# egorchistov/color-transfer

Hardware: AMD Instinct MI355X
Metric: stereopairs/s at 1920×1080 (linear + dcmcs3di fwd), 1/2/4/8 GPU (higher is better)
Workload: dtype f32 (float32 I/O; float32 difference forms in both sweeps, float64 only in the per-frame statistics records)

## Files before the change

### color-transfer_amd/csrc/reinhard_persist.hip

```cpp
#include <atomic>
#include <mutex>

#include "ct_reinhard.h"
#include "ct_reinhard_persist.h"

namespace ct {
namespace rp {

#ifndef CT_RP_ILP
#define CT_RP_ILP 1
#endif
#define CT_RP_PIXEL_FENCE(q) do { if (((q) + 1) % CT_RP_ILP == 0) __builtin_amdgcn_sched_barrier(0); } while (0)

#ifndef CT_RP_F32_WAVES
#define CT_RP_F32_WAVES 16
#endif
constexpr int kMaxWaves = 16;
constexpr int kTileBytes = kTilePixels * 12;
constexpr int kShards = 8;
constexpr int kRecWords = 32;
constexpr int kDataWords = 24;
constexpr int kSlabWord = 24;
constexpr int kMaxPairs = 64;
constexpr int kErrBytes = 64;

constexpr uint64_t kValMask = (1ull << 52) - 1;
constexpr int kInvShift = 52, kCntShift = 58;
constexpr double kHiScale = 0x1p24, kLoScale = 0x1p40;
constexpr int64_t kHiBias = 1ll << 46;

struct Scratch {
    double red[2][kMaxWaves][12];
    double coef[2][8];
    double side[kMaxWaves][6];
    double tot[12];
    double stat[2][CT_LAB_STATS_STRIDE];
    double fin[12 * 8];
    unsigned long long rec[kShards * kDataWords];
    float piv[2 * kMaxPairs][4];
    float lut255[256];
    float lin255f[256];
    unsigned cnt[2];
    unsigned ticket[3];
    unsigned ready[2];
    int flag[2];
};
constexpr int kLdsFixed = lut::kLdsBytesAll + (int)sizeof(Scratch);
constexpr int kLdsMax = 160 * 1024;
constexpr int kMaxParked = (kLdsMax - kLdsFixed) / (2 * kTileBytes);
constexpr int kMaxSlots = 32 * kMaxWaves / 2;
static_assert(lut::kLdsBytesAll % 16 == 0 && kTileBytes % 16 == 0, "16-byte aligned LDS regions");

struct Args {
    const void *target, *reference, *gt;
    float *out;
    int64_t n_pixels;
    int batch, slots, pslots;
    unsigned long long *rec;
    double *slab;
    double *sq;
    unsigned *err;
    double *stats_t, *stats_r;
    unsigned long long *stamps;
};

__device__ __forceinline__ uint64_t realtime() { return __builtin_amdgcn_s_memrealtime(); }
constexpr uint64_t kSpinTicks = 200000000ull;
__device__ unsigned g_status;
__device__ __forceinline__ void give_up(unsigned *err) {
    __hip_atomic_store(err, 1u, __ATOMIC_RELAXED, __HIP_MEMORY_SCOPE_AGENT);
    (void)__hip_atomic_fetch_or(&g_status, 1u, __ATOMIC_RELAXED, __HIP_MEMORY_SCOPE_AGENT);
}

template <typename T> struct Tile;
template <> struct Tile<float> {
    struct Raw { float e[12]; };
    static __device__ __forceinline__ void load(const void *p, int lane, Raw &r) { load_tile(reinterpret_cast<const float *>(p), lane, r.e); }
    static __device__ __forceinline__ bool in_range(const Raw &r) { return __builtin_amdgcn_ballot_w64(max_bits12(r.e) > lut::kOneBits) == 0; }
};
template <> struct Tile<uint8_t> {
    struct Raw { uint32_t d[3]; };
    static __device__ __forceinline__ void load(const void *p, int lane, Raw &r) {
        const uint8_t *q = reinterpret_cast<const uint8_t *>(p) + lane * 12;
        if ((reinterpret_cast<uintptr_t>(p) & 3) == 0) {
            typedef uint32_t u3 __attribute__((ext_vector_type(3)));
            const u3 v = *reinterpret_cast<const u3 __attribute__((aligned(4))) *>(q);
            r.d[0] = v.x; r.d[1] = v.y; r.d[2] = v.z;
        } else {
#pragma unroll
            for (int i = 0; i < 3; ++i) r.d[i] = (uint32_t)q[4 * i] | ((uint32_t)q[4 * i + 1] << 8) | ((uint32_t)q[4 * i + 2] << 16) | ((uint32_t)q[4 * i + 3] << 24);
        }
    }
    static __device__ __forceinline__ bool in_range(const Raw &) { return true; }
};
__device__ __forceinline__ uint32_t byte_of(const uint32_t (&d)[3], int i) { return (d[i >> 2] >> (8 * (i & 3))) & 255u; }

template <typename T>
__device__ __forceinline__ void load_pixel(const T *p, double &r, double &g, double &b) {
    if constexpr (sizeof(T) == 4) { r = p[0]; g = p[1]; b = p[2]; }
    else { r = (float)p[0] / 255.0f; g = (float)p[1] / 255.0f; b = (float)p[2] / 255.0f; }
}
template <typename T> __device__ __forceinline__ int pixel_of(int lane, int q) { return sizeof(T) == 4 ? q * kWave + lane : lane * 4 + q; }

template <typename T>
__device__ __forceinline__ void exact_moments_tile(const T *tile, const float (&kf)[3], double *side, int lane) {
    const double kd[3] = {(double)kf[0], (double)kf[1], (double)kf[2]};
    double s[6] = {0.0, 0.0, 0.0, 0.0, 0.0, 0.0};
#pragma unroll 1
    for (int q = 0; q < 4; ++q) {
        double r, g, b, x, y, z;
        load_pixel<T>(tile + pixel_of<T>(lane, q) * 3, r, g, b);
        to_space<true>(r, g, b, x, y, z);
        accumulate<true>(s, kd, x, y, z);
    }
#pragma unroll 1
    for (int m = 0; m < 6; ++m) {
        const double v = wave_sum(s[m]);
        if (lane == 0) side[m] += v;
    }
}

template <typename T, bool PARK, bool STATS = true>
__device__ __forceinline__ bool fwd_tile(const unsigned char *tab, Scratch *sc, const void *tile, typename Tile<T>::Raw &cur, const float (&kf)[3],
                                         float (&sf)[6], uint32_t *slot, int w, int lane) {
    const bool raw = !Tile<T>::in_range(cur);
    if constexpr (sizeof(T) == 4) {
        if (raw) {
            if (STATS) exact_moments_tile<T>(reinterpret_cast<const T *>(tile), kf, &sc->side[w][0], lane);
            return true;
        }
    }
    bool near = false;
#pragma unroll
    for (int q = 0; q < 4; ++q) {
        float fy, dxy, dyz;
        if constexpr (!PARK) {
            if constexpr (sizeof(T) == 4) {
                lut::rgb_to_f_stats(tab, cur.e[3 * q], cur.e[3 * q + 1], cur.e[3 * q + 2], fy, dxy, dyz);
            } else {
                const float l[3] = {sc->lin255f[byte_of(cur.d, 3 * q)], sc->lin255f[byte_of(cur.d, 3 * q + 1)], sc->lin255f[byte_of(cur.d, 3 * q + 2)]};
                lut::lin_to_f_stats(tab, l, fy, dxy, dyz);
            }
        } else {
            if constexpr (sizeof(T) == 4) {
                near |= lut::rgb_to_f(tab, cur.e[3 * q], cur.e[3 * q + 1], cur.e[3 * q + 2], fy, dxy, dyz);
            } else {
                const float l[3] = {sc->lin255f[byte_of(cur.d, 3 * q)], sc->lin255f[byte_of(cur.d, 3 * q + 1)], sc->lin255f[byte_of(cur.d, 3 * q + 2)]};
                near |= lut::lin_to_f(tab, l, fy, dxy, dyz);
            }
        }
        if (STATS) {
            const float e0 = fy - kf[0], e1 = dxy - kf[1], e2 = dyz - kf[2];
            sf[0] += e0; sf[1] += e1; sf[2] += e2;
            sf[3] = fmaf(e0, e0, sf[3]); sf[4] = fmaf(e1, e1, sf[4]); sf[5] = fmaf(e2, e2, sf[5]);
        }
        if (PARK) {
            slot[(3 * q) * kWave + lane] = __float_as_uint(fy);
            slot[(3 * q + 1) * kWave + lane] = __float_as_uint(dxy);
            slot[(3 * q + 2) * kWave + lane] = __float_as_uint(dyz);
        }
        CT_RP_PIXEL_FENCE(q);
    }
    return PARK && __builtin_amdgcn_ballot_w64(near) != 0;
}

template <typename T> __device__ __forceinline__ void store_pixel(float *tile, int lane, int q, float r, float g, float b) {
#ifdef CT_NT_STORE
    if constexpr (sizeof(T) == 4) {
        __builtin_nontemporal_store(float3v{r, g, b}, reinterpret_cast<float3u *>(tile + pixel_of<T>(lane, q) * 3));
        return;
    }
#endif
    *reinterpret_cast<float3u *>(tile + pixel_of<T>(lane, q) * 3) = float3v{r, g, b};
}

template <typename T, bool HAS_GT>
__device__ __forceinline__ void apply_tile(const unsigned char *tab, const Scratch *sc, const uint32_t *slot, bool raw, bool coef_bad,
                                           const ReinhardCoef &c, const float (&cf)[6], const void *tgt_tile, const void *gt_tile,
                                           float *out_tile, const typename Tile<T>::Raw &gv, double &sq, int lane) {
    float e = 0.f;
    auto gt_of = [&](int i) -> float {
        if constexpr (sizeof(T) == 4) return gv.e[i]; else return sc->lut255[byte_of(gv.d, i)];
    };
    bool slow = raw || coef_bad;
    if (!slow) {
        bool near = false;
#pragma unroll
        for (int q = 0; q < 4; ++q) {
            const float fy = __uint_as_float(slot[(3 * q) * kWave + lane]), dxy = __uint_as_float(slot[(3 * q + 1) * kWave + lane]),
                        dyz = __uint_as_float(slot[(3 * q + 2) * kWave + lane]);
            const float gy = fmaf(cf[0], fy, cf[3]), dx = fmaf(cf[1], dxy, cf[4]), dz = fmaf(cf[2], dyz, cf[5]);
            float r, g, b;
            near |= lut::f_to_rgb_clip(tab, gy, dx, dz, r, g, b);
            store_pixel<T>(out_tile, lane, q, r, g, b);
            if (HAS_GT) {
                const float d0 = r - gt_of(3 * q), d1 = g - gt_of(3 * q + 1), d2 = b - gt_of(3 * q + 2);
                e = fmaf(d0, d0, e); e = fmaf(d1, d1, e); e = fmaf(d2, d2, e);
            }
            CT_RP_PIXEL_FENCE(q);
        }
        slow = __builtin_amdgcn_ballot_w64(near) != 0;
    }
    if (slow) {
        e = 0.f;
#pragma unroll 1
        for (int q = 0; q < 4; ++q) {
            const int px = pixel_of<T>(lane, q);
            double r, g, b;
            load_pixel<T>(reinterpret_cast<const T *>(tgt_tile) + px * 3, r, g, b);
            float o0, o1, o2;
            reinhard_pixel<float, false>(c, r, g, b, o0, o1, o2);
            *reinterpret_cast<float3u *>(out_tile + px * 3) = float3v{o0, o1, o2};
            if (HAS_GT) {
                double g0, g1, g2;
                load_pixel<T>(reinterpret_cast<const T *>(gt_tile) + px * 3, g0, g1, g2);
                const float d0 = o0 - (float)g0, d1 = o1 - (float)g1, d2 = o2 - (float)g2;
                e = fmaf(d0, d0, e); e = fmaf(d1, d1, e); e = fmaf(d2, d2, e);
            }
        }
    }
    if (HAS_GT) sq += (double)e;
}

__device__ __forceinline__ int collect(const unsigned long long *rec, int nwg, int lane, Scratch *sc, unsigned *err) {
    const uint64_t t0 = realtime();
    for (;;) {
        bool ok = true;
#pragma unroll
        for (int j = 0; j < 3; ++j) {
            const int idx = lane + kWave * j;
            const int shard = idx / kDataWords, q = idx - shard * kDataWords;
            const unsigned long long x = __hip_atomic_load(rec + shard * kRecWords + q, __ATOMIC_RELAXED, __HIP_MEMORY_SCOPE_AGENT);
            ok &= (x >> kCntShift) == (unsigned long long)((nwg - shard + kShards - 1) / kShards);
            sc->rec[idx] = x;
        }
        __threadfence_block();
        if (__builtin_amdgcn_ballot_w64(!ok) == 0) break;
        if (realtime() - t0 > kSpinTicks) { if (lane == 0) give_up(err); return 2; }
        __builtin_amdgcn_s_sleep(8);
    }
    unsigned long long val = 0, inv = 0;
    if (lane < kDataWords) {
#pragma unroll
        for (int s = 0; s < kShards; ++s) {
            const unsigned long long x = sc->rec[s * kDataWords + lane];
            val += x & kValMask;
            inv += (x >> kInvShift) & 63ull;
        }
    }
    double dv = (lane & 1) ? (double)val * 0x1p-64 : (double)((long long)val - (long long)nwg * kHiBias) * 0x1p-24;
    dv += __shfl_down(dv, 1, kWave);
    if (lane < kDataWords && !(lane & 1)) sc->tot[lane >> 1] = dv;
    __threadfence_block();
    return __builtin_amdgcn_ballot_w64(lane < kDataWords && inv != 0) ? 1 : 0;
}

__device__ __forceinline__ void finish_stats(Scratch *sc, int par, int pair, int batch, int64_t n_pixels, int lane, double *stats_t, double *stats_r) {
    const double n = (double)n_pixels;
    if (lane < 6) {
        const int img = lane / 3, ch = lane - 3 * img;
        const double s1 = sc->tot[img * 6 + ch], s2 = sc->tot[img * 6 + 3 + ch];
        const double k = (double)sc->piv[img ? batch + pair : pair][ch];
        const double m0 = s1 / n;
        const double var = fma(-s1, m0, s2) / n;
        const double scale = ch == 0 ? 116.0 : (ch == 1 ? 500.0 : 200.0);
        const double mean = ch == 0 ? fma(116.0, k + m0, -16.0) : scale * (k + m0);
        const double sd = scale * var_to_sd(var, kVarFloorF32);
        sc->stat[img][ch] = mean;
        sc->stat[img][3 + ch] = sd;
        if (ch == 0) { sc->stat[img][6] = n; sc->stat[img][7] = 0.0; }
    }
    __threadfence_block();
    if (lane < 3) {
        const double mt = sc->stat[0][lane], st = sc->stat[0][3 + lane], mr = sc->stat[1][lane], sr = sc->stat[1][3 + lane];
        const double s = sr / st;
        double off;
        if (lane == 0) off = (fma(-16.0 - mt, s, mr) + 16.0) * (1.0 / 116.0);
        else off = fma(-mt, s, mr) * (lane == 1 ? 1.0 / 500.0 : 1.0 / 200.0);
        sc->coef[par][lane] = s;
        sc->coef[par][3 + lane] = off;
    }
    if (stats_t != nullptr && lane < 2 * CT_LAB_STATS_STRIDE) {
        const int img = lane / CT_LAB_STATS_STRIDE, m = lane - img * CT_LAB_STATS_STRIDE;
        (img ? stats_r : stats_t)[(size_t)pair * CT_LAB_STATS_STRIDE + m] = sc->stat[img][m];
    }
}

__device__ __forceinline__ float uniform_f32(float v) { return __uint_as_float(__builtin_amdgcn_readfirstlane(__float_as_uint(v))); }

template <typename T>
__device__ __forceinline__ void tail_moments(const T *p, int tail, const float (&kf)[3], Scratch *sc, int w, int lane) {
    if (w * kWave >= tail) return;
    double s[6] = {0.0, 0.0, 0.0, 0.0, 0.0, 0.0};
    const int t = w * kWave + lane;
    if (t < tail) {
        const double kd[3] = {(double)kf[0], (double)kf[1], (double)kf[2]};
        double x, y, z, r0, r1, r2;
        if constexpr (sizeof(T) == 4) { r0 = p[t * 3]; r1 = p[t * 3 + 1]; r2 = p[t * 3 + 2]; }
        else { r0 = (float)p[t * 3] / 255.0f; r1 = (float)p[t * 3 + 1] / 255.0f; r2 = (float)p[t * 3 + 2] / 255.0f; }
        to_space<true>(r0, r1, r2, x, y, z);
        accumulate<true>(s, kd, x, y, z);
    }
#pragma unroll 1
    for (int m = 0; m < 6; ++m) {
        const double v = wave_sum(s[m]);
        if (lane == 0) sc->side[w][m] += v;
    }
}

template <typename T, bool HAS_GT, int kWaves>
__global__ __launch_bounds__(kWaves * kWave) void reinhard_persist_kernel(const Args a) {
    constexpr int kThreads = kWaves * kWave;
    extern __shared__ __attribute__((aligned(16))) unsigned char smem[];
    unsigned char *tab = smem;
    uint32_t *park = reinterpret_cast<uint32_t *>(smem + lut::kLdsBytesAll);
    Scratch *sc = reinterpret_cast<Scratch *>(smem + lut::kLdsBytesAll + (size_t)2 * a.pslots * kTileBytes);
    const int lane = threadIdx.x & (kWave - 1);
    const int w = __builtin_amdgcn_readfirstlane(threadIdx.x >> 6);
    const int g = blockIdx.x, nwg = gridDim.x;
    const int B = a.batch;
    const int64_t n_full = a.n_pixels / kTilePixels;
    constexpr size_t kPx = 3 * sizeof(T);
    int Kw = 0;
    for (int s = w; s < a.slots && (int64_t)s * nwg + g < n_full; s += kWaves) ++Kw;
    const int tail = (g == nwg - 1) ? (int)(a.n_pixels - n_full * kTilePixels) : 0;
    const int n_stages = 2 + 2 * B;

    auto parked = [&](int k) -> bool { return w + kWaves * k < a.pslots; };
    auto slot_of = [&](int p, int k) -> uint32_t * { return park + ((size_t)(p & 1) * a.pslots + (w + kWaves * k)) * (kTileBytes / 4); };
    auto tile_off = [&](int k) -> size_t { return (size_t)((int64_t)(w + kWaves * k) * nwg + g) * kTilePixels; };
    auto tile_ptr = [&](const void *base, int pair, int k) -> const void * {
        return reinterpret_cast<const unsigned char *>(base) + ((size_t)pair * a.n_pixels + tile_off(k)) * kPx;
    };
    auto stage_pair = [&](int st) -> int { return (st < 2 || (st & 1)) ? (st == 0 ? 0 : (st + 1) >> 1) : (st - 2) >> 1; };
    auto is_sweep = [&](int st) -> bool { return st < 2 || (st & 1); };
    auto job_exists = [&](int st, int j) -> bool {
        const int p = stage_pair(st);
        if (p >= B) return false;
        if (is_sweep(st)) return true;
        return (j & 1) ? HAS_GT : !parked(j >> 1);
    };
    auto job_ptr = [&](int st, int j) -> const void * {
        const int p = stage_pair(st);
        if (is_sweep(st)) return j < Kw ? tile_ptr(a.reference, p, j) : tile_ptr(a.target, p, j - Kw);
        return (j & 1) ? tile_ptr(a.gt, p, j >> 1) : tile_ptr(a.target, p, j >> 1);
    };
    auto next_load = [&](int st, int j) -> const void * {
        if (Kw == 0) return nullptr;
        do {
            if (++j >= 2 * Kw) { j = 0; ++st; }
        } while (st < n_stages && !job_exists(st, j));
        return st < n_stages ? job_ptr(st, j) : nullptr;
    };

    typename Tile<T>::Raw cur, nxt;
    if (Kw > 0 && B > 0) Tile<T>::load(job_ptr(0, 0), lane, cur);
    lut::load_tables<kThreads, true>(tab);
    float p0[3] = {0.5f, 0.5f, 0.5f};
    const bool piv_thread = threadIdx.x < 2 * B && a.n_pixels > 0;
    if (piv_thread) {
        const int img = threadIdx.x;
        const T *p = reinterpret_cast<const T *>(img < B ? a.target : a.reference) + (size_t)(img < B ? img : img - B) * a.n_pixels * 3;
        if constexpr (sizeof(T) == 4) { p0[0] = p[0]; p0[1] = p[1]; p0[2] = p[2]; }
        else { p0[0] = (float)p[0] / 255.0f; p0[1] = (float)p[1] / 255.0f; p0[2] = (float)p[2] / 255.0f; }
    }
    if (threadIdx.x < 2) { sc->cnt[threadIdx.x] = 0; sc->flag[threadIdx.x] = 0; sc->ready[threadIdx.x] = 0; }
    if (threadIdx.x < 3) sc->ticket[threadIdx.x] = 0;
    if (sizeof(T) == 1 && threadIdx.x < 256) sc->lut255[threadIdx.x] = (float)threadIdx.x / 255.0f;
    __syncthreads();
    if (sizeof(T) == 1 && threadIdx.x < 256) {
        sc->lin255f[threadIdx.x] = lut::expand(tab, sc->lut255[threadIdx.x]);
    }
    if (threadIdx.x < 2 * B) {
        float fy = 0.5f, dxy = 0.0f, dyz = 0.0f;
        if (piv_thread && max(max(__float_as_uint(p0[0]), __float_as_uint(p0[1])), __float_as_uint(p0[2])) <= lut::kOneBits) {
            lut::rgb_to_f_stats(tab, p0[0], p0[1], p0[2], fy, dxy, dyz);
        }
        sc->piv[threadIdx.x][0] = rintf(fy * 1024.0f) * (1.0f / 1024.0f);
        sc->piv[threadIdx.x][1] = rintf(dxy * 1024.0f) * (1.0f / 1024.0f);
        sc->piv[threadIdx.x][2] = rintf(dyz * 1024.0f) * (1.0f / 1024.0f);
    }
    __syncthreads();

    uint32_t rawmask0 = 0, rawmask1 = 0;
#ifdef CT_RP_STAMPS
#define CT_RP_STAMP(slot) do { if (a.stamps && lane == 0 && (w == 0 || w == kWaves - 1)) \
        a.stamps[(((size_t)g * 2 + (w ? 1 : 0)) * n_stages + st) * 4 + (slot)] = realtime(); } while (0)
#else
#define CT_RP_STAMP(slot) do { } while (0)
#endif
    for (int st = 0; st < n_stages; ++st) {
        const int p = stage_pair(st), par = p & 1;
        if (p >= B) continue;
        CT_RP_STAMP(0);
        if (is_sweep(st)) {
            {
                float sf[6] = {0.f, 0.f, 0.f, 0.f, 0.f, 0.f};
                const float kf[3] = {uniform_f32(sc->piv[B + p][0]), uniform_f32(sc->piv[B + p][1]), uniform_f32(sc->piv[B + p][2])};
                if (lane < 6) sc->side[w][lane] = 0.0;
                for (int k = 0; k < Kw; ++k) {
                    const void *np = next_load(st, k);
                    if (np) Tile<T>::load(np, lane, nxt);
                    fwd_tile<T, false>(tab, sc, tile_ptr(a.reference, p, k), cur, kf, sf, nullptr, w, lane);
                    cur = nxt;
                }
                if (tail > 0) tail_moments(reinterpret_cast<const T *>(a.reference) + ((size_t)p * a.n_pixels + n_full * kTilePixels) * 3, tail, kf, sc, w, lane);
#pragma unroll
                for (int m = 0; m < 6; ++m) {
                    const float v = wave_sum_f32(sf[m]);
                    if (lane == 0) sc->red[par][w][6 + m] = (double)v + sc->side[w][m];
                }
            }
            CT_RP_STAMP(1);
            {
                float sf[6] = {0.f, 0.f, 0.f, 0.f, 0.f, 0.f};
                const float kf[3] = {uniform_f32(sc->piv[p][0]), uniform_f32(sc->piv[p][1]), uniform_f32(sc->piv[p][2])};
                if (lane < 6) sc->side[w][lane] = 0.0;
                uint32_t rm = 0;
                for (int k = 0; k < Kw; ++k) {
                    const void *np = next_load(st, Kw + k);
                    if (np) Tile<T>::load(np, lane, nxt);
                    if (parked(k)) {
                        if (fwd_tile<T, true>(tab, sc, tile_ptr(a.target, p, k), cur, kf, sf, slot_of(p, k), w, lane)) rm |= 1u << k;
                    } else {
                        fwd_tile<T, false>(tab, sc, tile_ptr(a.target, p, k), cur, kf, sf, nullptr, w, lane);
                    }
                    cur = nxt;
                }
                if (par) rawmask1 = rm; else rawmask0 = rm;
                if (tail > 0) tail_moments(reinterpret_cast<const T *>(a.target) + ((size_t)p * a.n_pixels + n_full * kTilePixels) * 3, tail, kf, sc, w, lane);
#pragma unroll
                for (int m = 0; m < 6; ++m) {
                    const float v = wave_sum_f32(sf[m]);
                    if (lane == 0) sc->red[par][w][m] = (double)v + sc->side[w][m];
                }
            }
            CT_RP_STAMP(2);
            unsigned old = 0;
            if (lane == 0) {
                __threadfence_block();
                old = atomicAdd(&sc->cnt[par], 1u);
            }
            old = __builtin_amdgcn_readfirstlane(old);
            if (old == kWaves - 1) {
                __threadfence_block();
                double v = 0.0;
                if (lane < 12) {
                    v = sc->red[par][0][lane];
#pragma unroll
                    for (int ww = 1; ww < kWaves; ++ww) v += sc->red[par][ww][lane];
                }
                if (lane == 0) sc->cnt[par] = 0;
                const double vm = __shfl(v, lane >> 1, kWave);
                const bool fits = fabs(vm) < 0x1p22;
                if (lane < kDataWords) {
                    const double sc24 = (fits ? vm : 0.0) * kHiScale;
                    const double fl = floor(sc24);
                    const unsigned long long hi = (unsigned long long)((long long)fl + kHiBias);
                    const unsigned long long lo = (unsigned long long)((sc24 - fl) * kLoScale);
                    const unsigned long long word = ((lane & 1) ? lo : hi) + (1ull << kCntShift) + (fits ? 0ull : (1ull << kInvShift));
                    (void)__hip_atomic_fetch_add(a.rec + ((size_t)p * kShards + (g % kShards)) * kRecWords + lane, word, __ATOMIC_RELAXED,
                                                 __HIP_MEMORY_SCOPE_AGENT);
                }
                if (lane < 12)
                    __hip_atomic_store(reinterpret_cast<unsigned long long *>(a.slab + ((size_t)p * nwg + g) * 12 + lane),
                                       (unsigned long long)__double_as_longlong(v), __ATOMIC_RELAXED, __HIP_MEMORY_SCOPE_AGENT);
                asm volatile("s_waitcnt vmcnt(0)" ::: "memory");
                if (lane == 0)
                    (void)__hip_atomic_fetch_add(a.rec + ((size_t)p * kShards + (g % kShards)) * kRecWords + kSlabWord, 1ull, __ATOMIC_RELAXED,
                                                 __HIP_MEMORY_SCOPE_AGENT);
            }
            CT_RP_STAMP(3);
            continue;
        }
        bool timed_out = false;
        {
            unsigned tk = 0;
            if (lane == 0) tk = atomicAdd(&sc->ticket[p % 3], 1u);
            tk = __builtin_amdgcn_readfirstlane(tk);
            if (tk == 0) {
                const int rc0 = collect(a.rec + (size_t)p * kShards * kRecWords, nwg, lane, sc, a.err);
                if (rc0 == 0) finish_stats(sc, par, p, B, a.n_pixels, lane, g == 0 ? a.stats_t : nullptr, a.stats_r);
                if (lane == 0) {
                    sc->flag[par] = rc0;
                    __threadfence_block();
                    __hip_atomic_store(&sc->ready[par], (unsigned)(p + 1), __ATOMIC_RELEASE, __HIP_MEMORY_SCOPE_WORKGROUP);
                }
                CT_RP_STAMP(1);
            }
            if (tk == kWaves - 1 && lane == 0) sc->ticket[p % 3] = 0;
            bool ready_ok = true;
            const uint64_t tw = realtime();
            while (__hip_atomic_load(&sc->ready[par], __ATOMIC_ACQUIRE, __HIP_MEMORY_SCOPE_WORKGROUP) != (unsigned)(p + 1)) {
                if (realtime() - tw > 2 * kSpinTicks) { ready_ok = false; if (lane == 0) give_up(a.err); break; }
                __builtin_amdgcn_s_sleep(8);
            }
            if (!ready_ok) timed_out = true;
        }
        CT_RP_STAMP(2);
        const int rc = timed_out ? 2 : sc->flag[par];
        if (rc == 1) {
            if (threadIdx.x < 96) {
                const uint64_t t0 = realtime();
                for (;;) {
                    unsigned long long x = 0, want = 0;
                    if (lane < kShards) {
                        want = (unsigned long long)((nwg - lane + kShards - 1) / kShards);
                        x = __hip_atomic_load(a.rec + ((size_t)p * kShards + lane) * kRecWords + kSlabWord, __ATOMIC_RELAXED, __HIP_MEMORY_SCOPE_AGENT);
                    }
                    if (__builtin_amdgcn_ballot_w64(x != want) == 0) break;
                    if (realtime() - t0 > kSpinTicks) { if (lane == 0) give_up(a.err); break; }
                    __builtin_amdgcn_s_sleep(8);
                }
                __builtin_amdgcn_fence(__ATOMIC_ACQUIRE, "agent");
                const int m = threadIdx.x >> 3, sub = threadIdx.x & 7;
                const double *src = a.slab + (size_t)p * nwg * 12 + m;
                double acc = 0.0;
                for (int b = sub; b < nwg; b += 8) acc += src[(size_t)b * 12];
                sc->fin[m * 8 + sub] = acc;
            }
            __syncthreads();
            if (threadIdx.x < 12) {
                const double *f = sc->fin + threadIdx.x * 8;
                sc->tot[threadIdx.x] = ((((((f[0] + f[1]) + f[2]) + f[3]) + f[4]) + f[5]) + f[6]) + f[7];
            }
            __syncthreads();
            if (w == 0) finish_stats(sc, par, p, B, a.n_pixels, lane, g == 0 ? a.stats_t : nullptr, a.stats_r);
            __syncthreads();
        }
        ReinhardCoef c;
        c.sL = uniform_f64(sc->coef[par][0]); c.sa = uniform_f64(sc->coef[par][1]); c.sb = uniform_f64(sc->coef[par][2]);
        c.cy = uniform_f64(sc->coef[par][3]); c.ca = uniform_f64(sc->coef[par][4]); c.cb = uniform_f64(sc->coef[par][5]);
        if (rc == 2) { c.sL = c.sa = c.sb = c.cy = c.ca = c.cb = __longlong_as_double(0x7ff8000000000000ll); }
        const bool coef_bad = !reinhard_coef_fast(c);
        const float cf[6] = {(float)c.sL, (float)c.sa, (float)c.sb, (float)c.cy, (float)c.ca, (float)c.cb};
        double sq = 0.0;
        const uint32_t rawmask = par ? rawmask1 : rawmask0;
        for (int k = 0; k < Kw; ++k) {
            const size_t off = (size_t)p * a.n_pixels + tile_off(k);
            const void *tgt_tile = reinterpret_cast<const unsigned char *>(a.target) + off * kPx;
            const void *gt_tile = HAS_GT ? reinterpret_cast<const unsigned char *>(a.gt) + off * kPx : nullptr;
            const uint32_t *slot = slot_of(p, k);
            bool raw = (rawmask >> k) & 1u;
            if (!parked(k)) {
                const void *np = next_load(st, 2 * k);
                if (np) Tile<T>::load(np, lane, nxt);
                float none[6];
                const float kz[3] = {0.f, 0.f, 0.f};
                uint32_t *tmp = slot_of(p, 0);
                raw = fwd_tile<T, true, false>(tab, sc, tgt_tile, cur, kz, none, tmp, w, lane);
                slot = tmp;
                cur = nxt;
            }
            if (HAS_GT) {
                const void *np = next_load(st, 2 * k + 1);
                if (np) Tile<T>::load(np, lane, nxt);
            }
            apply_tile<T, HAS_GT>(tab, sc, slot, raw, coef_bad, c, cf, tgt_tile, gt_tile, a.out + off * 3, cur, sq, lane);
            if (HAS_GT) cur = nxt;
        }
        if ((int)threadIdx.x < tail) {
            const size_t px = (size_t)p * a.n_pixels + n_full * kTilePixels + threadIdx.x;
            double r0, r1, r2;
            load_pixel<T>(reinterpret_cast<const T *>(a.target) + px * 3, r0, r1, r2);
            float o0, o1, o2;
            reinhard_pixel<float, false>(c, r0, r1, r2, o0, o1, o2);
            a.out[px * 3] = o0; a.out[px * 3 + 1] = o1; a.out[px * 3 + 2] = o2;
            if (HAS_GT) {
                double g0, g1, g2;
                load_pixel<T>(reinterpret_cast<const T *>(a.gt) + px * 3, g0, g1, g2);
                const double d0 = (double)o0 - g0, d1 = (double)o1 - g1, d2 = (double)o2 - g2;
                sq += (d0 * d0 + d1 * d1) + d2 * d2;
            }
        }
        if (HAS_GT) {
            const double v = wave_sum(sq);
            if (kWaves < kMaxWaves && lane == 0) a.sq[((size_t)p * nwg + g) * kMaxWaves + kWaves + w] = 0.0;
            if (lane == 0) a.sq[((size_t)p * nwg + g) * kMaxWaves + w] = v;
        }
        CT_RP_STAMP(3);
    }
}

__global__ __launch_bounds__(256) void psnr_finish_persist_kernel(const double *__restrict__ sq, int n_parts, int64_t n_elems, double *__restrict__ out,
                                                                  const unsigned *__restrict__ err) {
    __shared__ double lds[4];
    double s[1] = {0.0};
    for (int i = threadIdx.x; i < n_parts; i += 256) s[0] += sq[(size_t)blockIdx.x * n_parts + i];
    block_sum<1>(s, lds);
    if (threadIdx.x == 0) {
        double mse = s[0] / (double)n_elems;
        if (*err != 0u) mse = __longlong_as_double(0x7ff8000000000000ll);
        out[blockIdx.x * 2] = mse;
        out[blockIdx.x * 2 + 1] = 10.0 * log10(1.0 / (mse > 1e-300 ? mse : (mse == mse ? 1e-300 : mse)));
    }
}

constexpr int kMaxGrid = 63 * kShards;
static int grid_size() {
    static std::atomic<int> cache[kMaxDevices];
    const int dev = current_device();
    int n = cache[dev].load(std::memory_order_relaxed);
    if (n == 0) {
        int cus = 256;
        (void)hipDeviceGetAttribute(&cus, hipDeviceAttributeMultiprocessorCount, dev);
        (void)hipGetLastError();
        n = cus > 0 ? cus : 256;
        const int forced = env_int("CT_HIP_PERSIST_WGS", 0);
        if (forced > 0 && forced <= n) n = forced;
        if (n > kMaxGrid) n = -1;
        cache[dev].store(n, std::memory_order_relaxed);
    }
    return n > 0 ? n : 0;
}
static int slots_for(int64_t n_pixels) {
    const int64_t tiles = n_pixels / kTilePixels;
    const int g = grid_size();
    if (g <= 0) return kMaxSlots + 1;
    return (int)((tiles + g - 1) / g);
}

bool eligible(int64_t n_pixels, bool any_size) {
    static const bool on = [] { const char *e = env_str("CT_HIP_REINHARD_PERSIST"); return e && e[0] == '1'; }();
    if (n_pixels < kTilePixels) return false;
    const int slots = slots_for(n_pixels);
    if (slots > kMaxSlots) return false;
    if (any_size) return true;
    return on && slots >= kMaxWaves && slots <= 2 * kMaxParked;
}

static size_t rec_bytes(int batch) { return kErrBytes + (size_t)batch * kShards * kRecWords * sizeof(unsigned long long); }

size_t ws_bytes(int64_t n_pixels, int batch) {
    if (!eligible(n_pixels, true) || batch <= 0) return 0;
    const int b = batch < kMaxPairs ? batch : kMaxPairs;
    const size_t g = (size_t)grid_size();
    size_t n = rec_bytes(b) + (size_t)b * g * 12 * sizeof(double) + (size_t)b * g * kMaxWaves * sizeof(double);
#ifdef CT_RP_STAMPS
    n += g * 2 * (size_t)(2 + 2 * b) * 4 * sizeof(unsigned long long);
#endif
    return n;
}

static std::mutex g_chain_mutex;
static hipEvent_t g_chain_event[kMaxDevices];
static hipStream_t g_chain_stream[kMaxDevices];

static int f32_waves() {
    static const int v = [] { const int x = env_int("CT_HIP_PERSIST_WAVES", 0); return x == 8 || x == 16 ? x : CT_RP_F32_WAVES; }();
    return v;
}

bool overlaps(const float *out, const void *target, const void *reference, const void *gt, int64_t n_pixels, int batch, size_t elem_bytes) {
    const uintptr_t o0 = reinterpret_cast<uintptr_t>(out), o1 = o0 + (size_t)batch * n_pixels * 3 * sizeof(float);
    const size_t in_bytes = (size_t)batch * n_pixels * 3 * elem_bytes;
    for (const void *q : {target, reference, gt}) {
        const uintptr_t q0 = reinterpret_cast<uintptr_t>(q);
        if (q != nullptr && q0 < o1 && o0 < q0 + in_bytes) return true;
    }
    return false;
}

template <typename T>
int launch(const T *target, const T *reference, const T *gt, float *out, double *psnr_out, int64_t n_pixels, int batch, double *stats_out,
           void *ws, size_t ws_size, hipStream_t stream, hipEvent_t ev_start, hipEvent_t ev_stop) {
    if (!eligible(n_pixels, true)) return CT_E_BADARG;
    if (ws == nullptr || (reinterpret_cast<uintptr_t>(ws) & 15) || ws_size < ws_bytes(n_pixels, batch)) return CT_E_WORKSPACE;
    if (gt != nullptr && psnr_out == nullptr) return CT_E_BADARG;
    if (overlaps(out, target, reference, gt, n_pixels, batch, sizeof(T))) return CT_E_BADARG;
    const int g = grid_size();
    const int slots = slots_for(n_pixels);
    const int pslots = slots < kMaxParked ? slots : kMaxParked;
    const size_t lds = (size_t)kLdsFixed + (size_t)2 * pslots * kTileBytes;
    int waves = kMaxWaves;
    void (*kern)(const Args) = gt ? reinhard_persist_kernel<T, true, kMaxWaves> : reinhard_persist_kernel<T, false, kMaxWaves>;
    if constexpr (sizeof(T) == 4) {
        if (f32_waves() == 8) {
            waves = 8;
            kern = gt ? reinhard_persist_kernel<T, true, 8> : reinhard_persist_kernel<T, false, 8>;
        }
    }
    static DynLdsAttr attr[4];
    const int dev = current_device();
    {
        hipError_t e = attr[(gt ? 1 : 0) + (waves == 8 ? 2 : 0)].ensure(reinterpret_cast<const void *>(kern), kLdsMax);
        if (e != hipSuccess) return (int)e;
    }
    hipStreamCaptureStatus cap = hipStreamCaptureStatusNone;
    (void)hipStreamIsCapturing(stream, &cap);
    (void)hipGetLastError();
    const bool chain = cap == hipStreamCaptureStatusNone;
    hipEvent_t *const chain_event = g_chain_event;
    hipStream_t *const chain_stream = g_chain_stream;
    std::unique_lock<std::mutex> chain_lock(g_chain_mutex, std::defer_lock);
    if (chain) {
        chain_lock.lock();
        if (chain_event[dev] == nullptr) {
            if (hipEventCreateWithFlags(&chain_event[dev], hipEventDisableTiming) != hipSuccess) { (void)hipGetLastError(); chain_event[dev] = nullptr; }
        } else if (chain_stream[dev] != stream) {
            (void)hipStreamWaitEvent(stream, chain_event[dev], 0);
        }
    }
    for (int b0 = 0; b0 < batch; b0 += kMaxPairs) {
        const int b = batch - b0 < kMaxPairs ? batch - b0 : kMaxPairs;
        Args a;
        a.target = target + (size_t)b0 * n_pixels * 3;
        a.reference = reference + (size_t)b0 * n_pixels * 3;
        a.gt = gt ? gt + (size_t)b0 * n_pixels * 3 : nullptr;
        a.out = out + (size_t)b0 * n_pixels * 3;
        a.n_pixels = n_pixels; a.batch = b; a.slots = slots; a.pslots = pslots;
        unsigned char *base = reinterpret_cast<unsigned char *>(ws);
        a.err = reinterpret_cast<unsigned *>(base);
        a.rec = reinterpret_cast<unsigned long long *>(base + kErrBytes);
        a.slab = reinterpret_cast<double *>(base + rec_bytes(b));
        a.sq = a.slab + (size_t)b * g * 12;
#ifdef CT_RP_STAMPS
        a.stamps = reinterpret_cast<unsigned long long *>(a.sq + (size_t)b * g * kMaxWaves);
#else
        a.stamps = nullptr;
#endif
        a.stats_t = stats_out ? stats_out + (size_t)b0 * CT_LAB_STATS_STRIDE : nullptr;
        a.stats_r = stats_out ? stats_out + (size_t)(batch + b0) * CT_LAB_STATS_STRIDE : nullptr;
        { const int zr = zero_async(base, rec_bytes(b), stream); if (zr) return zr; }
        if (ev_start && b0 == 0) (void)hipEventRecord(ev_start, stream);
        hipLaunchKernelGGL(kern, dim3(g), dim3(waves * kWave), lds, stream, a);
        CT_CHECK_LAUNCH();
        if (ev_stop && b0 + b >= batch) (void)hipEventRecord(ev_stop, stream);
        if (gt) {
            hipLaunchKernelGGL(psnr_finish_persist_kernel, dim3(b), dim3(256), 0, stream, (const double *)a.sq, g * kMaxWaves, n_pixels * 3,
                               psnr_out + (size_t)b0 * 2, (const unsigned *)a.err);
            CT_CHECK_LAUNCH();
        }
    }
    if (chain && chain_event[dev] != nullptr) {
        (void)hipEventRecord(chain_event[dev], stream);
        chain_stream[dev] = stream;
    }
    return CT_OK;
}

int read_status(bool clear) {
    unsigned v = 0;
    if (hipMemcpyFromSymbol(&v, HIP_SYMBOL(g_status), sizeof(v), 0, hipMemcpyDeviceToHost) != hipSuccess) { (void)hipGetLastError(); return -1; }
    if (clear && v != 0) {
        const unsigned z = 0;
        (void)hipMemcpyToSymbol(HIP_SYMBOL(g_status), &z, sizeof(z), 0, hipMemcpyHostToDevice);
    }
    return (int)(v & 1u);
}

template int launch<float>(const float *, const float *, const float *, float *, double *, int64_t, int, double *, void *, size_t, hipStream_t,
                           hipEvent_t, hipEvent_t);
template int launch<uint8_t>(const uint8_t *, const uint8_t *, const uint8_t *, float *, double *, int64_t, int, double *, void *, size_t,
                             hipStream_t, hipEvent_t, hipEvent_t);

}
}
```

Baseline: 41790.

## Interleave apply of previous pair with sweeps of next pair in persistent kernel

After: 41760. No clear change (-0.1%).

```diff
diff --git a/color-transfer_amd/csrc/reinhard_persist.hip b/color-transfer_amd/csrc/reinhard_persist.hip
--- a/color-transfer_amd/csrc/reinhard_persist.hip
+++ b/color-transfer_amd/csrc/reinhard_persist.hip
@@ -323,38 +323,39 @@
     constexpr size_t kPx = 3 * sizeof(T);
     int Kw = 0;
     for (int s = w; s < a.slots && (int64_t)s * nwg + g < n_full; s += kWaves) ++Kw;
+    const int Kp = min(Kw, a.pslots > w ? (a.pslots - w + kWaves - 1) / kWaves : 0);
     const int tail = (g == nwg - 1) ? (int)(a.n_pixels - n_full * kTilePixels) : 0;
-    const int n_stages = 2 + 2 * B;
-
-    auto parked = [&](int k) -> bool { return w + kWaves * k < a.pslots; };
+    [[maybe_unused]] const int n_stages = 2 + 2 * B;
+
     auto slot_of = [&](int p, int k) -> uint32_t * { return park + ((size_t)(p & 1) * a.pslots + (w + kWaves * k)) * (kTileBytes / 4); };
-    auto tile_off = [&](int k) -> size_t { return (size_t)((int64_t)(w + kWaves * k) * nwg + g) * kTilePixels; };
-    auto tile_ptr = [&](const void *base, int pair, int k) -> const void * {
-        return reinterpret_cast<const unsigned char *>(base) + ((size_t)pair * a.n_pixels + tile_off(k)) * kPx;
+    const size_t px_wave = ((size_t)w * nwg + g) * kTilePixels, px_stride = (size_t)kWaves * nwg * kTilePixels;
+    auto tile_px = [&](int pair, int k) -> size_t { return (size_t)pair * a.n_pixels + px_wave + (size_t)k * px_stride; };
+    auto tile_ptr = [&](const void *base, int pair, int k) -> const unsigned char * {
+        return reinterpret_cast<const unsigned char *>(base) + tile_px(pair, k) * kPx;
     };
-    auto stage_pair = [&](int st) -> int { return (st < 2 || (st & 1)) ? (st == 0 ? 0 : (st + 1) >> 1) : (st - 2) >> 1; };
-    auto is_sweep = [&](int st) -> bool { return st < 2 || (st & 1); };
-    auto job_exists = [&](int st, int j) -> bool {
-        const int p = stage_pair(st);
-        if (p >= B) return false;
-        if (is_sweep(st)) return true;
-        return (j & 1) ? HAS_GT : !parked(j >> 1);
+    constexpr bool kAlwaysLoad = sizeof(T) == 4;
+    constexpr int kPosT = 1, kPosA = 2;
+    auto first_load = [&](int pos, int i) -> const unsigned char * {
+        if (pos == kPosA) {
+            if (i < 1) return nullptr;
+            if (Kp == 0) return tile_ptr(a.target, i - 1, 0);
+            if (HAS_GT) return tile_ptr(a.gt, i - 1, 0);
+            return Kp < Kw ? tile_ptr(a.target, i - 1, Kp) : nullptr;
+        }
+        if (i >= B) return nullptr;
+        return tile_ptr(pos == kPosT ? a.target : a.reference, i, 0);
     };
-    auto job_ptr = [&](int st, int j) -> const void * {
-        const int p = stage_pair(st);
-        if (is_sweep(st)) return j < Kw ? tile_ptr(a.reference, p, j) : tile_ptr(a.target, p, j - Kw);
-        return (j & 1) ? tile_ptr(a.gt, p, j >> 1) : tile_ptr(a.target, p, j >> 1);
+    auto load_after = [&](int pos, int i) -> const unsigned char * {
+        for (;;) {
+            if (++pos == 3) { pos = 0; ++i; }
+            if (i > B) return kAlwaysLoad ? tile_ptr(a.reference, 0, 0) : nullptr;
+            const unsigned char *q = first_load(pos, i);
+            if (q != nullptr) return q;
+        }
     };
-    auto next_load = [&](int st, int j) -> const void * {
-        if (Kw == 0) return nullptr;
-        do {
-            if (++j >= 2 * Kw) { j = 0; ++st; }
-        } while (st < n_stages && !job_exists(st, j));
-        return st < n_stages ? job_ptr(st, j) : nullptr;
-    };
 
     typename Tile<T>::Raw cur, nxt;
-    if (Kw > 0 && B > 0) Tile<T>::load(job_ptr(0, 0), lane, cur);
+    if (Kw > 0 && B > 0) Tile<T>::load(tile_ptr(a.reference, 0, 0), lane, cur);
     lut::load_tables<kThreads, true>(tab);
     float p0[3] = {0.5f, 0.5f, 0.5f};
     const bool piv_thread = threadIdx.x < 2 * B && a.n_pixels > 0;
@@ -384,58 +385,195 @@
 
     uint32_t rawmask0 = 0, rawmask1 = 0;
 #ifdef CT_RP_STAMPS
-#define CT_RP_STAMP(slot) do { if (a.stamps && lane == 0 && (w == 0 || w == kWaves - 1)) \
-        a.stamps[(((size_t)g * 2 + (w ? 1 : 0)) * n_stages + st) * 4 + (slot)] = realtime(); } while (0)
+#define CT_RP_STAMP(st, slot) do { if (a.stamps && lane == 0 && (w == 0 || w == kWaves - 1)) \
+        a.stamps[(((size_t)g * 2 + (w ? 1 : 0)) * n_stages + (st)) * 4 + (slot)] = realtime(); } while (0)
 #else
-#define CT_RP_STAMP(slot) do { } while (0)
+#define CT_RP_STAMP(st, slot) do { } while (0)
 #endif
-    for (int st = 0; st < n_stages; ++st) {
-        const int p = stage_pair(st), par = p & 1;
-        if (p >= B) continue;
-        CT_RP_STAMP(0);
-        if (is_sweep(st)) {
-            {
-                float sf[6] = {0.f, 0.f, 0.f, 0.f, 0.f, 0.f};
-                const float kf[3] = {uniform_f32(sc->piv[B + p][0]), uniform_f32(sc->piv[B + p][1]), uniform_f32(sc->piv[B + p][2])};
-                if (lane < 6) sc->side[w][lane] = 0.0;
-                for (int k = 0; k < Kw; ++k) {
-                    const void *np = next_load(st, k);
-                    if (np) Tile<T>::load(np, lane, nxt);
-                    fwd_tile<T, false>(tab, sc, tile_ptr(a.reference, p, k), cur, kf, sf, nullptr, w, lane);
-                    cur = nxt;
+
+    auto apply_phase = [&](const int p, const int round) {
+        const int par = p & 1;
+        const int st = 2 * p + 2;
+        (void)st;
+        CT_RP_STAMP(st, 0);
+        bool timed_out = false;
+        {
+            unsigned tk = 0;
+            if (lane == 0) tk = atomicAdd(&sc->ticket[p % 3], 1u);
+            tk = __builtin_amdgcn_readfirstlane(tk);
+            if (tk == 0) {
+                const int rc0 = collect(a.rec + (size_t)p * kShards * kRecWords, nwg, lane, sc, a.err);
+                if (rc0 == 0) finish_stats(sc, par, p, B, a.n_pixels, lane, g == 0 ? a.stats_t : nullptr, a.stats_r);
+                if (lane == 0) {
+                    sc->flag[par] = rc0;
+                    __threadfence_block();
+                    __hip_atomic_store(&sc->ready[par], (unsigned)(p + 1), __ATOMIC_RELEASE, __HIP_MEMORY_SCOPE_WORKGROUP);
                 }
-                if (tail > 0) tail_moments(reinterpret_cast<const T *>(a.reference) + ((size_t)p * a.n_pixels + n_full * kTilePixels) * 3, tail, kf, sc, w, lane);
+                CT_RP_STAMP(st, 1);
+            }
+            if (tk == kWaves - 1 && lane == 0) sc->ticket[p % 3] = 0;
+            bool ready_ok = true;
+            const uint64_t tw = realtime();
+            while (__hip_atomic_load(&sc->ready[par], __ATOMIC_ACQUIRE, __HIP_MEMORY_SCOPE_WORKGROUP) != (unsigned)(p + 1)) {
+                if (realtime() - tw > 2 * kSpinTicks) { ready_ok = false; if (lane == 0) give_up(a.err); break; }
+                __builtin_amdgcn_s_sleep(8);
+            }
+            if (!ready_ok) timed_out = true;
+        }
+        CT_RP_STAMP(st, 2);
+        const int rc = timed_out ? 2 : sc->flag[par];
+        if (rc == 1) {
+            if (threadIdx.x < 96) {
+                const uint64_t t0 = realtime();
+                for (;;) {
+                    unsigned long long x = 0, want = 0;
+                    if (lane < kShards) {
+                        want = (unsigned long long)((nwg - lane + kShards - 1) / kShards);
+                        x = __hip_atomic_load(a.rec + ((size_t)p * kShards + lane) * kRecWords + kSlabWord, __ATOMIC_RELAXED, __HIP_MEMORY_SCOPE_AGENT);
+                    }
+                    if (__builtin_amdgcn_ballot_w64(x != want) == 0) break;
+                    if (realtime() - t0 > kSpinTicks) { if (lane == 0) give_up(a.err); break; }
+                    __builtin_amdgcn_s_sleep(8);
+                }
+                __builtin_amdgcn_fence(__ATOMIC_ACQUIRE, "agent");
+                const int m = threadIdx.x >> 3, sub = threadIdx.x & 7;
+                const double *src = a.slab + (size_t)p * nwg * 12 + m;
+                double acc = 0.0;
+                for (int b = sub; b < nwg; b += 8) acc += src[(size_t)b * 12];
+                sc->fin[m * 8 + sub] = acc;
+            }
+            __syncthreads();
+            if (threadIdx.x < 12) {
+                const double *f = sc->fin + threadIdx.x * 8;
+                sc->tot[threadIdx.x] = ((((((f[0] + f[1]) + f[2]) + f[3]) + f[4]) + f[5]) + f[6]) + f[7];
+            }
+            __syncthreads();
+            if (w == 0) finish_stats(sc, par, p, B, a.n_pixels, lane, g == 0 ? a.stats_t : nullptr, a.stats_r);
+            __syncthreads();
+        }
+        ReinhardCoef c;
+        c.sL = uniform_f64(sc->coef[par][0]); c.sa = uniform_f64(sc->coef[par][1]); c.sb = uniform_f64(sc->coef[par][2]);
+        c.cy = uniform_f64(sc->coef[par][3]); c.ca = uniform_f64(sc->coef[par][4]); c.cb = uniform_f64(sc->coef[par][5]);
+        if (rc == 2) { c.sL = c.sa = c.sb = c.cy = c.ca = c.cb = __longlong_as_double(0x7ff8000000000000ll); }
+        const bool coef_bad = !reinhard_coef_fast(c);
+        const float cf[6] = {(float)c.sL, (float)c.sa, (float)c.sb, (float)c.cy, (float)c.ca, (float)c.cb};
+        double sq = 0.0;
+        const uint32_t rawmask = par ? rawmask1 : rawmask0;
+        size_t off = tile_px(p, 0);
+#pragma unroll 1
+        for (int k = 0; k < Kw; ++k, off += px_stride) {
+            const unsigned char *tgt_tile = reinterpret_cast<const unsigned char *>(a.target) + off * kPx;
+            const unsigned char *gt_tile = HAS_GT ? reinterpret_cast<const unsigned char *>(a.gt) + off * kPx : nullptr;
+            const uint32_t *slot = slot_of(p, k);
+            bool raw = (rawmask >> k) & 1u;
+            const bool last = k + 1 >= Kw;
+            if (k >= Kp) {
+                const unsigned char *np = HAS_GT ? gt_tile : (last ? load_after(kPosA, round) : tgt_tile + px_stride * kPx);
+                if (kAlwaysLoad || np) Tile<T>::load(np, lane, nxt);
+                float none[6];
+                const float kz[3] = {0.f, 0.f, 0.f};
+                uint32_t *tmp = slot_of(p, 0);
+                raw = fwd_tile<T, true, false>(tab, sc, tgt_tile, cur, kz, none, tmp, w, lane);
+                slot = tmp;
+                cur = nxt;
+            }
+            if (HAS_GT) {
+                const unsigned char *np = last ? load_after(kPosA, round) : (k + 1 >= Kp ? tgt_tile : gt_tile) + px_stride * kPx;
+                if (kAlwaysLoad || np) Tile<T>::load(np, lane, nxt);
+            }
+            apply_tile<T, HAS_GT>(tab, sc, slot, raw, coef_bad, c, cf, tgt_tile, gt_tile, a.out + off * 3, cur, sq, lane);
+            if (HAS_GT) cur = nxt;
+        }
+        if ((int)threadIdx.x < tail) {
+            const size_t px = (size_t)p * a.n_pixels + n_full * kTilePixels + threadIdx.x;
+            double r0, r1, r2;
+            load_pixel<T>(reinterpret_cast<const T *>(a.target) + px * 3, r0, r1, r2);
+            float o0, o1, o2;
+            reinhard_pixel<float, false>(c, r0, r1, r2, o0, o1, o2);
+            a.out[px * 3] = o0; a.out[px * 3 + 1] = o1; a.out[px * 3 + 2] = o2;
+            if (HAS_GT) {
+                double g0, g1, g2;
+                load_pixel<T>(reinterpret_cast<const T *>(a.gt) + px * 3, g0, g1, g2);
+                const double d0 = (double)o0 - g0, d1 = (double)o1 - g1, d2 = (double)o2 - g2;
+                sq += (d0 * d0 + d1 * d1) + d2 * d2;
+            }
+        }
+        if (HAS_GT) {
+            const double v = wave_sum(sq);
+            if (kWaves < kMaxWaves && lane == 0) a.sq[((size_t)p * nwg + g) * kMaxWaves + kWaves + w] = 0.0;
+            if (lane == 0) a.sq[((size_t)p * nwg + g) * kMaxWaves + w] = v;
+        }
+        CT_RP_STAMP(st, 3);
+    };
+
+    for (int i = 0; i <= B; ++i) {
+        const int p = i, par = p & 1;
+        const int st = p < 2 ? p : 2 * p - 1;
+        (void)st;
+        if (i < B) {
+            CT_RP_STAMP(st, 0);
+            float sf[6] = {0.f, 0.f, 0.f, 0.f, 0.f, 0.f};
+            const float kf[3] = {uniform_f32(sc->piv[B + p][0]), uniform_f32(sc->piv[B + p][1]), uniform_f32(sc->piv[B + p][2])};
+            if (lane < 6) sc->side[w][lane] = 0.0;
+            const unsigned char *tp = tile_ptr(a.reference, p, 0);
+            auto r_tile = [&](typename Tile<T>::Raw &use, typename Tile<T>::Raw &fill, int k) {
+                const unsigned char *np = k + 1 < Kw ? tp + px_stride * kPx : load_after(0, i);
+                if (kAlwaysLoad || np) Tile<T>::load(np, lane, fill);
+                fwd_tile<T, false>(tab, sc, tp, use, kf, sf, nullptr, w, lane);
+                tp += px_stride * kPx;
+            };
+            if constexpr (sizeof(T) == 4) {
+#pragma unroll 1
+                for (int k = 0; k < Kw; k += 2) {
+                    r_tile(cur, nxt, k);
+                    if (k + 1 < Kw) r_tile(nxt, cur, k + 1); else cur = nxt;
+                }
+            } else {
+#pragma unroll 1
+                for (int k = 0; k < Kw; ++k) { r_tile(cur, nxt, k); cur = nxt; }
+            }
+            if (tail > 0) tail_moments(reinterpret_cast<const T *>(a.reference) + ((size_t)p * a.n_pixels + n_full * kTilePixels) * 3, tail, kf, sc, w, lane);
 #pragma unroll
-                for (int m = 0; m < 6; ++m) {
-                    const float v = wave_sum_f32(sf[m]);
-                    if (lane == 0) sc->red[par][w][6 + m] = (double)v + sc->side[w][m];
+            for (int m = 0; m < 6; ++m) {
+                const float v = wave_sum_f32(sf[m]);
+                if (lane == 0) sc->red[par][w][6 + m] = (double)v + sc->side[w][m];
+            }
+            CT_RP_STAMP(st, 1);
+        }
+        if (i < B) {
+            float sf[6] = {0.f, 0.f, 0.f, 0.f, 0.f, 0.f};
+            const float kf[3] = {uniform_f32(sc->piv[p][0]), uniform_f32(sc->piv[p][1]), uniform_f32(sc->piv[p][2])};
+            if (lane < 6) sc->side[w][lane] = 0.0;
+            uint32_t rm = 0;
+            const unsigned char *tp = tile_ptr(a.target, p, 0);
+            auto t_tile = [&](typename Tile<T>::Raw &use, typename Tile<T>::Raw &fill, int k) {
+                const unsigned char *np = k + 1 < Kw ? tp + px_stride * kPx : load_after(kPosT, i);
+                if (kAlwaysLoad || np) Tile<T>::load(np, lane, fill);
+                if (k < Kp) {
+                    if (fwd_tile<T, true>(tab, sc, tp, use, kf, sf, slot_of(p, k), w, lane)) rm |= 1u << k;
+                } else {
+                    fwd_tile<T, false>(tab, sc, tp, use, kf, sf, nullptr, w, lane);
                 }
-            }
-            CT_RP_STAMP(1);
-            {
-                float sf[6] = {0.f, 0.f, 0.f, 0.f, 0.f, 0.f};
-                const float kf[3] = {uniform_f32(sc->piv[p][0]), uniform_f32(sc->piv[p][1]), uniform_f32(sc->piv[p][2])};
-                if (lane < 6) sc->side[w][lane] = 0.0;
-                uint32_t rm = 0;
-                for (int k = 0; k < Kw; ++k) {
-                    const void *np = next_load(st, Kw + k);
-                    if (np) Tile<T>::load(np, lane, nxt);
-                    if (parked(k)) {
-                        if (fwd_tile<T, true>(tab, sc, tile_ptr(a.target, p, k), cur, kf, sf, slot_of(p, k), w, lane)) rm |= 1u << k;
-                    } else {
-                        fwd_tile<T, false>(tab, sc, tile_ptr(a.target, p, k), cur, kf, sf, nullptr, w, lane);
-                    }
-                    cur = nxt;
+                tp += px_stride * kPx;
+            };
+            if constexpr (sizeof(T) == 4) {
+#pragma unroll 1
+                for (int k = 0; k < Kw; k += 2) {
+                    t_tile(cur, nxt, k);
+                    if (k + 1 < Kw) t_tile(nxt, cur, k + 1); else cur = nxt;
                 }
-                if (par) rawmask1 = rm; else rawmask0 = rm;
-                if (tail > 0) tail_moments(reinterpret_cast<const T *>(a.target) + ((size_t)p * a.n_pixels + n_full * kTilePixels) * 3, tail, kf, sc, w, lane);
+            } else {
+#pragma unroll 1
+                for (int k = 0; k < Kw; ++k) { t_tile(cur, nxt, k); cur = nxt; }
+            }
+            if (par) rawmask1 = rm; else rawmask0 = rm;
+            if (tail > 0) tail_moments(reinterpret_cast<const T *>(a.target) + ((size_t)p * a.n_pixels + n_full * kTilePixels) * 3, tail, kf, sc, w, lane);
 #pragma unroll
-                for (int m = 0; m < 6; ++m) {
-                    const float v = wave_sum_f32(sf[m]);
-                    if (lane == 0) sc->red[par][w][m] = (double)v + sc->side[w][m];
-                }
-            }
-            CT_RP_STAMP(2);
+            for (int m = 0; m < 6; ++m) {
+                const float v = wave_sum_f32(sf[m]);
+                if (lane == 0) sc->red[par][w][m] = (double)v + sc->side[w][m];
+            }
+            CT_RP_STAMP(st, 2);
             unsigned old = 0;
             if (lane == 0) {
                 __threadfence_block();
@@ -470,115 +608,9 @@
                     (void)__hip_atomic_fetch_add(a.rec + ((size_t)p * kShards + (g % kShards)) * kRecWords + kSlabWord, 1ull, __ATOMIC_RELAXED,
                                                  __HIP_MEMORY_SCOPE_AGENT);
             }
-            CT_RP_STAMP(3);
-            continue;
-        }
-        bool timed_out = false;
-        {
-            unsigned tk = 0;
-            if (lane == 0) tk = atomicAdd(&sc->ticket[p % 3], 1u);
-            tk = __builtin_amdgcn_readfirstlane(tk);
-            if (tk == 0) {
-                const int rc0 = collect(a.rec + (size_t)p * kShards * kRecWords, nwg, lane, sc, a.err);
-                if (rc0 == 0) finish_stats(sc, par, p, B, a.n_pixels, lane, g == 0 ? a.stats_t : nullptr, a.stats_r);
-                if (lane == 0) {
-                    sc->flag[par] = rc0;
-                    __threadfence_block();
-                    __hip_atomic_store(&sc->ready[par], (unsigned)(p + 1), __ATOMIC_RELEASE, __HIP_MEMORY_SCOPE_WORKGROUP);
-                }
-                CT_RP_STAMP(1);
-            }
-            if (tk == kWaves - 1 && lane == 0) sc->ticket[p % 3] = 0;
-            bool ready_ok = true;
-            const uint64_t tw = realtime();
-            while (__hip_atomic_load(&sc->ready[par], __ATOMIC_ACQUIRE, __HIP_MEMORY_SCOPE_WORKGROUP) != (unsigned)(p + 1)) {
-                if (realtime() - tw > 2 * kSpinTicks) { ready_ok = false; if (lane == 0) give_up(a.err); break; }
-                __builtin_amdgcn_s_sleep(8);
-            }
-            if (!ready_ok) timed_out = true;
-        }
-        CT_RP_STAMP(2);
-        const int rc = timed_out ? 2 : sc->flag[par];
-        if (rc == 1) {
-            if (threadIdx.x < 96) {
-                const uint64_t t0 = realtime();
-                for (;;) {
-                    unsigned long long x = 0, want = 0;
-                    if (lane < kShards) {
-                        want = (unsigned long long)((nwg - lane + kShards - 1) / kShards);
-                        x = __hip_atomic_load(a.rec + ((size_t)p * kShards + lane) * kRecWords + kSlabWord, __ATOMIC_RELAXED, __HIP_MEMORY_SCOPE_AGENT);
-                    }
-                    if (__builtin_amdgcn_ballot_w64(x != want) == 0) break;
-                    if (realtime() - t0 > kSpinTicks) { if (lane == 0) give_up(a.err); break; }
-                    __builtin_amdgcn_s_sleep(8);
-                }
-                __builtin_amdgcn_fence(__ATOMIC_ACQUIRE, "agent");
-                const int m = threadIdx.x >> 3, sub = threadIdx.x & 7;
-                const double *src = a.slab + (size_t)p * nwg * 12 + m;
-                double acc = 0.0;
-                for (int b = sub; b < nwg; b += 8) acc += src[(size_t)b * 12];
-                sc->fin[m * 8 + sub] = acc;
-            }
-            __syncthreads();
-            if (threadIdx.x < 12) {
-                const double *f = sc->fin + threadIdx.x * 8;
-                sc->tot[threadIdx.x] = ((((((f[0] + f[1]) + f[2]) + f[3]) + f[4]) + f[5]) + f[6]) + f[7];
-            }
-            __syncthreads();
-            if (w == 0) finish_stats(sc, par, p, B, a.n_pixels, lane, g == 0 ? a.stats_t : nullptr, a.stats_r);
-            __syncthreads();
-        }
-        ReinhardCoef c;
-        c.sL = uniform_f64(sc->coef[par][0]); c.sa = uniform_f64(sc->coef[par][1]); c.sb = uniform_f64(sc->coef[par][2]);
-        c.cy = uniform_f64(sc->coef[par][3]); c.ca = uniform_f64(sc->coef[par][4]); c.cb = uniform_f64(sc->coef[par][5]);
-        if (rc == 2) { c.sL = c.sa = c.sb = c.cy = c.ca = c.cb = __longlong_as_double(0x7ff8000000000000ll); }
-        const bool coef_bad = !reinhard_coef_fast(c);
-        const float cf[6] = {(float)c.sL, (float)c.sa, (float)c.sb, (float)c.cy, (float)c.ca, (float)c.cb};
-        double sq = 0.0;
-        const uint32_t rawmask = par ? rawmask1 : rawmask0;
-        for (int k = 0; k < Kw; ++k) {
-            const size_t off = (size_t)p * a.n_pixels + tile_off(k);
-            const void *tgt_tile = reinterpret_cast<const unsigned char *>(a.target) + off * kPx;
-            const void *gt_tile = HAS_GT ? reinterpret_cast<const unsigned char *>(a.gt) + off * kPx : nullptr;
-            const uint32_t *slot = slot_of(p, k);
-            bool raw = (rawmask >> k) & 1u;
-            if (!parked(k)) {
-                const void *np = next_load(st, 2 * k);
-                if (np) Tile<T>::load(np, lane, nxt);
-                float none[6];
-                const float kz[3] = {0.f, 0.f, 0.f};
-                uint32_t *tmp = slot_of(p, 0);
-                raw = fwd_tile<T, true, false>(tab, sc, tgt_tile, cur, kz, none, tmp, w, lane);
-                slot = tmp;
-                cur = nxt;
-            }
-            if (HAS_GT) {
-                const void *np = next_load(st, 2 * k + 1);
-                if (np) Tile<T>::load(np, lane, nxt);
-            }
-            apply_tile<T, HAS_GT>(tab, sc, slot, raw, coef_bad, c, cf, tgt_tile, gt_tile, a.out + off * 3, cur, sq, lane);
-            if (HAS_GT) cur = nxt;
-        }
-        if ((int)threadIdx.x < tail) {
-            const size_t px = (size_t)p * a.n_pixels + n_full * kTilePixels + threadIdx.x;
-            double r0, r1, r2;
-            load_pixel<T>(reinterpret_cast<const T *>(a.target) + px * 3, r0, r1, r2);
-            float o0, o1, o2;
-            reinhard_pixel<float, false>(c, r0, r1, r2, o0, o1, o2);
-            a.out[px * 3] = o0; a.out[px * 3 + 1] = o1; a.out[px * 3 + 2] = o2;
-            if (HAS_GT) {
-                double g0, g1, g2;
-                load_pixel<T>(reinterpret_cast<const T *>(a.gt) + px * 3, g0, g1, g2);
-                const double d0 = (double)o0 - g0, d1 = (double)o1 - g1, d2 = (double)o2 - g2;
-                sq += (d0 * d0 + d1 * d1) + d2 * d2;
-            }
-        }
-        if (HAS_GT) {
-            const double v = wave_sum(sq);
-            if (kWaves < kMaxWaves && lane == 0) a.sq[((size_t)p * nwg + g) * kMaxWaves + kWaves + w] = 0.0;
-            if (lane == 0) a.sq[((size_t)p * nwg + g) * kMaxWaves + w] = v;
-        }
-        CT_RP_STAMP(3);
+            CT_RP_STAMP(st, 3);
+        }
+        if (i >= 1) apply_phase(i - 1, i);
     }
 }
 
```
